# zc402/video-classification

Hardware: AMD Instinct MI355X
Metric: clips/sec SlowFast-R50 8x8, 32x224^2 bf16 training step (higher is better)
Workload: dtype bf16

## Files before the change

### video-classification_amd/csrc/bn_tail.hip

```cpp
#include "sfk_common.h"

namespace {

template <typename D> __device__ __forceinline__ float wload(const void* w, int64_t i) {
  return (float)static_cast<const D*>(w)[i];
}

constexpr int TF_CO = 8;
constexpr int TF_MAXC = 512;

__global__ __launch_bounds__(256) void bn_tail_fold_g_kernel(const float* __restrict__ parts, int nparts, int c, float* __restrict__ g) {
  const int ci = blockIdx.x * 4 + (threadIdx.x >> 6), lane = threadIdx.x & 63;
  if (ci >= c) return;
  double s = 0.0;
  for (int p = lane; p < nparts; p += 64) s += (double)parts[((int64_t)p * c + ci) * 2];
#pragma unroll
  for (int sft = 1; sft < 64; sft <<= 1) s += __shfl_xor(s, sft);
  if (lane == 0) g[ci] = (float)s;
}

template <typename D>
__global__ __launch_bounds__(256) void bn_tail_fwd_kernel(const float* __restrict__ gram, const float* __restrict__ gvec,
                                                          double n, int c, const void* w,
                                                          int cout, const float* gamma, const float* beta, float eps,
                                                          float momentum, float* running_mean, float* running_var,
                                                          int64_t* nbt, float* mean, float* invstd, float* scale,
                                                          float* shift, float* __restrict__ t, D* __restrict__ wd) {
  __shared__ float wl[TF_CO][TF_MAXC];
  __shared__ double gl[TF_MAXC];
  __shared__ double red[4 * TF_CO][2];
  __shared__ float acoef[TF_CO];
  const int co0 = blockIdx.x * TF_CO, tid = threadIdx.x;
  if (blockIdx.x == 0 && tid == 0 && nbt) nbt[0] += 1;
  const double inv_n = 1.0 / n;
  for (int i = tid; i < TF_CO * c; i += 256) {
    const int o = i / c, j = i % c;
    wl[o][j] = co0 + o < cout ? wload<D>(w, (int64_t)(co0 + o) * c + j) : 0.f;
  }
  for (int j = tid; j < c; j += 256) gl[j] = (double)gvec[j] * inv_n;
  __syncthreads();
  constexpr int NR = TF_MAXC / 256;
  float acc[TF_CO][NR], accc[TF_CO][NR];
  double gbar[NR];
#pragma unroll
  for (int r = 0; r < NR; ++r) {
    const int ci = tid + 256 * r;
    gbar[r] = ci < c ? (double)gvec[ci] * inv_n : 0.0;
  }
#pragma unroll
  for (int o = 0; o < TF_CO; ++o)
#pragma unroll
    for (int r = 0; r < NR; ++r) { acc[o][r] = 0.f; accc[o][r] = 0.f; }
#pragma unroll 8
  for (int j = 0; j < c; ++j) {
    float gj[NR], gc[NR];
    const double mj = gl[j];
#pragma unroll
    for (int r = 0; r < NR; ++r) {
      const int ci = tid + 256 * r;
      gj[r] = ci < c ? gram[(int64_t)j * c + ci] : 0.f;
      gc[r] = (float)((double)gj[r] * inv_n - mj * gbar[r]);
    }
#pragma unroll
    for (int o = 0; o < TF_CO; ++o) {
      const float wv = wl[o][j];
#pragma unroll
      for (int r = 0; r < NR; ++r) {
        acc[o][r] += wv * gj[r];
        accc[o][r] += wv * gc[r];
      }
    }
  }
  double p1[TF_CO], p2[TF_CO];
#pragma unroll
  for (int o = 0; o < TF_CO; ++o) {
    p1[o] = 0.0;
    p2[o] = 0.0;
#pragma unroll
    for (int r = 0; r < NR; ++r) {
      const int ci = tid + 256 * r;
      if (ci < c) {
        if (co0 + o < cout) t[(int64_t)(co0 + o) * c + ci] = acc[o][r];
        p1[o] += (double)wl[o][ci] * (double)gvec[ci];
        p2[o] += (double)accc[o][r] * (double)wl[o][ci];
      }
    }
#pragma unroll
    for (int sft = 1; sft < 64; sft <<= 1) {
      p1[o] += __shfl_xor(p1[o], sft);
      p2[o] += __shfl_xor(p2[o], sft);
    }
  }
  if ((tid & 63) == 0) {
#pragma unroll
    for (int o = 0; o < TF_CO; ++o) {
      red[(tid >> 6) * TF_CO + o][0] = p1[o];
      red[(tid >> 6) * TF_CO + o][1] = p2[o];
    }
  }
  __syncthreads();
  if (tid < TF_CO && co0 + tid < cout) {
    const int ch = co0 + tid;
    const double s1 = red[tid][0] + red[TF_CO + tid][0] + red[2 * TF_CO + tid][0] + red[3 * TF_CO + tid][0];
    const double s2 = red[tid][1] + red[TF_CO + tid][1] + red[2 * TF_CO + tid][1] + red[3 * TF_CO + tid][1];
    const double mu = s1 / n;
    double var = s2;
    if (var < 0.0) var = 0.0;
    const float is = (float)(1.0 / sqrt(var + (double)eps));
    const float sc = gamma[ch] * is;
    mean[ch] = (float)mu;
    invstd[ch] = is;
    scale[ch] = sc;
    shift[ch] = beta[ch] - (float)mu * sc;
    acoef[tid] = sc;
    if (running_mean) {
      const double unb = n > 1.0 ? var * n / (n - 1.0) : var;
      running_mean[ch] = (1.f - momentum) * running_mean[ch] + momentum * (float)mu;
      running_var[ch] = (1.f - momentum) * running_var[ch] + momentum * (float)unb;
    }
  }
  if (!wd) return;
  __syncthreads();
  for (int ci = tid; ci < c; ci += 256)
#pragma unroll
    for (int o = 0; o < TF_CO; ++o)
      if (co0 + o < cout) wd[(int64_t)ci * cout + co0 + o] = (D)(acoef[o] * wl[o][ci]);
}

template <typename D>
__global__ __launch_bounds__(256) void bn_tail_coef_kernel(const float* __restrict__ rx, const float* __restrict__ parts,
                                                           int nparts, double n, int c,
                                                           const void* w, int cout, const float* gamma,
                                                           const float* mean, const float* invstd, float* dgamma,
                                                           float* dbeta, float* coef) {
  const int co = blockIdx.x * 4 + (threadIdx.x >> 6), lane = threadIdx.x & 63;
  if (co >= cout) return;
  double sdy = 0.0;
#pragma unroll 4
  for (int ci = lane; ci < c; ci += 64) sdy += (double)wload<D>(w, (int64_t)co * c + ci) * (double)rx[(int64_t)co * c + ci];
  double s = 0.0;
#pragma unroll 8
  for (int p = lane; p < nparts; p += 64) s += (double)parts[((int64_t)p * cout + co) * 2];
#pragma unroll
  for (int sft = 1; sft < 64; sft <<= 1) {
    sdy += __shfl_xor(sdy, sft);
    s += __shfl_xor(s, sft);
  }
  if (lane != 0) return;
  const double is = (double)invstd[co], mu = (double)mean[co];
  const double sxh = is * (sdy - mu * s);
  dgamma[co] += (float)sxh;
  dbeta[co] += (float)s;
  const double A = (double)gamma[co] * is, c1 = s / n, c2 = sxh / n;
  coef[co * 4 + 0] = (float)A;
  coef[co * 4 + 1] = (float)(-A * c2 * is);
  coef[co * 4 + 2] = (float)(A * (c2 * is * mu - c1));
  coef[co * 4 + 3] = 0.f;
}

template <typename D>
__device__ __forceinline__ void bn_tail_apply_part(int bx, int by, const float* __restrict__ rx, const float* __restrict__ gvec,
                                                   const float* __restrict__ t, int c, int cout,
                                                   const float* __restrict__ coef, float* dw) {
  const int co0 = by * 32, ci0 = bx * 32;
  const int tx = threadIdx.x & 31, ty = threadIdx.x >> 5;
#pragma unroll
  for (int i = 0; i < 4; ++i) {
    const int co = co0 + ty + 8 * i, ci = ci0 + tx;
    if (co < cout && ci < c) {
      const float A = coef[co * 4], B = coef[co * 4 + 1], Cc = coef[co * 4 + 2];
      const int64_t idx = (int64_t)co * c + ci;
      dw[idx] += A * rx[idx] + B * t[idx] + Cc * gvec[ci];
    }
  }
}

template <typename D>
__device__ __forceinline__ void bn_tail_m_part(int bx, int by, const void* w, int c, int cout, const float* __restrict__ coef, D* m) {
  __shared__ float wi[16][17], wj[16][17], bco[16];
  const int tx = threadIdx.x & 15, ty = threadIdx.x >> 4;
  const int i = by * 16 + ty, j = bx * 16 + tx;
  float acc = 0.f;
  for (int co0 = 0; co0 < cout; co0 += 16) {
    const int co = co0 + ty;
    const int ci = by * 16 + tx, cj = bx * 16 + tx;
    wi[ty][tx] = (co < cout && ci < c) ? wload<D>(w, (int64_t)co * c + ci) : 0.f;
    wj[ty][tx] = (co < cout && cj < c) ? wload<D>(w, (int64_t)co * c + cj) : 0.f;
    if (threadIdx.x < 16) bco[threadIdx.x] = co0 + threadIdx.x < cout ? coef[(co0 + threadIdx.x) * 4 + 1] : 0.f;
    __syncthreads();
#pragma unroll
    for (int q = 0; q < 16; ++q) acc += bco[q] * wi[q][ty] * wj[q][tx];
    __syncthreads();
  }
  if (i < c && j < c) m[(int64_t)i * c + j] = (D)acc;
}

template <typename D>
__device__ __forceinline__ void bn_tail_bias_part(int bx, const void* w, int c, int cout, const float* __restrict__ coef,
                                                  float* bias) {
  __shared__ double red[16][17];
  const int col = threadIdx.x & 15, part = threadIdx.x >> 4;
  const int ci = bx * 16 + col;
  double s = 0.0;
  if (ci < c) {
#pragma unroll 4
    for (int co = part; co < cout; co += 16) s += (double)coef[co * 4 + 2] * (double)wload<D>(w, (int64_t)co * c + ci);
  }
  red[part][col] = s;
  __syncthreads();
  if (part == 0 && ci < c) {
    double a = 0.0;
#pragma unroll
    for (int p = 0; p < 16; ++p) a += red[p][col];
    bias[ci] = (float)a;
  }
}

template <typename D>
__global__ __launch_bounds__(256) void bn_tail_post_kernel(const float* rx, const float* gvec, const float* t, int c,
                                                           const void* w, int cout, const float* coef, float* dw, D* m,
                                                           float* bias, int ax, int nap, int mx, int nm) {
  int b = blockIdx.x;
  if (b < nap) { bn_tail_apply_part<D>(b % ax, b / ax, rx, gvec, t, c, cout, coef, dw); return; }
  b -= nap;
  if (b < nm) { bn_tail_m_part<D>(b % mx, b / mx, w, c, cout, coef, m); return; }
  bn_tail_bias_part<D>(b - nm, w, c, cout, coef, bias);
}

inline bool tail_args_ok(int c, int cout, int dtype) {
  return c > 0 && cout > 0 && (dtype == SFK_F32 || dtype == SFK_BF16);
}

}

extern "C" int sfk_bn_tail_fwd(const float* gram, const float* a_sums, int32_t a_nparts, int64_t count, float* g, int32_t c,
                               const void* w, int32_t w_dtype, int32_t cout,
                               const float* gamma, const float* beta, float eps, float momentum, float* running_mean,
                               float* running_var, int64_t* nbt, float* mean, float* invstd, float* scale, float* shift,
                               float* t, void* wd, sfk_stream_t stream) {
  if (!gram || !a_sums || a_nparts <= 0 || count <= 0 || !g || !w || !gamma || !beta || !mean || !invstd || !scale || !shift || !t)
    return SFK_ERR_INVALID;
  if (!tail_args_ok(c, cout, w_dtype) || (!running_mean) != (!running_var)) return SFK_ERR_INVALID;
  if (c > TF_MAXC) return SFK_ERR_UNSUPPORTED;
  hipStream_t s = static_cast<hipStream_t>(stream);
  hipLaunchKernelGGL(bn_tail_fold_g_kernel, dim3((c + 3) / 4), dim3(256), 0, s, a_sums, a_nparts, c, g);
  const dim3 grid((cout + TF_CO - 1) / TF_CO), blk(256);
  if (w_dtype == SFK_BF16)
    hipLaunchKernelGGL(bn_tail_fwd_kernel<bf16_t>, grid, blk, 0, s, gram, g, (double)count, c, w, cout, gamma, beta, eps, momentum,
                       running_mean, running_var, nbt, mean, invstd, scale, shift, t, static_cast<bf16_t*>(wd));
  else
    hipLaunchKernelGGL(bn_tail_fwd_kernel<float>, grid, blk, 0, s, gram, g, (double)count, c, w, cout, gamma, beta, eps, momentum,
                       running_mean, running_var, nbt, mean, invstd, scale, shift, t, static_cast<float*>(wd));
  SFK_CHECK_LAUNCH();
  return SFK_OK;
}

template <typename D>
static int tail_bwd_launch(const float* rx, const float* parts, int nparts, const float* g, int64_t count, const float* t, int c, const void* w, int cout,
                           const float* gamma, const float* mean, const float* invstd, float* dgamma, float* dbeta,
                           float* dw, void* m, float* bias, float* coef, hipStream_t s) {
  hipLaunchKernelGGL(bn_tail_coef_kernel<D>, dim3((cout + 3) / 4), dim3(256), 0, s, rx, parts, nparts, (double)count, c, w, cout, gamma, mean,
                     invstd, dgamma, dbeta, coef);
  const int ax = (c + 31) / 32, ay = (cout + 31) / 32, mx = (c + 15) / 16, nb = (c + 15) / 16;
  hipLaunchKernelGGL(bn_tail_post_kernel<D>, dim3(ax * ay + mx * mx + nb), dim3(256), 0, s, rx, g, t, c, w, cout, coef, dw,
                     static_cast<D*>(m), bias, ax, ax * ay, mx, mx * mx);
  SFK_CHECK_LAUNCH();
  return SFK_OK;
}

extern "C" int sfk_bn_tail_bwd(const float* rx, const float* parts, int32_t nparts, const float* g, int64_t count, const float* t,
                               int32_t c, const void* w, int32_t w_dtype, int32_t cout, const float* gamma, const float* mean, const float* invstd,
                               float* dgamma, float* dbeta, float* dw, void* m, float* bias, float* coef,
                               sfk_stream_t stream) {
  if (!rx || !parts || nparts <= 0 || !g || count <= 0 || !t || !w || !gamma || !mean || !invstd || !dgamma || !dbeta || !dw || !m || !bias || !coef)
    return SFK_ERR_INVALID;
  if (!tail_args_ok(c, cout, w_dtype)) return SFK_ERR_INVALID;
  hipStream_t s = static_cast<hipStream_t>(stream);
  return w_dtype == SFK_BF16
             ? tail_bwd_launch<bf16_t>(rx, parts, nparts, g, count, t, c, w, cout, gamma, mean, invstd, dgamma, dbeta, dw, m, bias, coef, s)
             : tail_bwd_launch<float>(rx, parts, nparts, g, count, t, c, w, cout, gamma, mean, invstd, dgamma, dbeta, dw, m, bias, coef, s);
}
```

Before: 1173.

## Fuse partial-sum fold into BN tail forward kernel and stage gram slabs in LDS

The forward tail kernel now folds the per-part channel sums itself when the part count is small, which removes a separate kernel launch. It stages the gram matrix through LDS in slabs with register prefetch, and uses dynamic shared memory with templated column groupings so smaller channel counts keep more threads busy. The backward coef kernel uses a shared fold routine, and the M-part kernel processes 64 output channels per tile instead of 16. Explicit fma and unfused operations pin down rounding, and the code grows more complex with more template variants.

New measurement: 1177, median of 6. About the same (+0.3%).

```diff
diff --git a/video-classification_amd/csrc/bn_tail.hip b/video-classification_amd/csrc/bn_tail.hip
--- a/video-classification_amd/csrc/bn_tail.hip
+++ b/video-classification_amd/csrc/bn_tail.hip
@@ -6,8 +6,59 @@
   return (float)static_cast<const D*>(w)[i];
 }
 
+__device__ __forceinline__ float unfused_mul_add(float a, float b, float c) {
+#pragma clang fp contract(off)
+  const float p = a * b;
+  return c + p;
+}
+__device__ __forceinline__ float unfused_add(float a, float b) {
+#pragma clang fp contract(off)
+  return a + b;
+}
+
 constexpr int TF_CO = 8;
 constexpr int TF_MAXC = 512;
+constexpr int TF_SLAB = 2048;
+constexpr int TF_FOLD_CW = 64;
+
+template <int CW>
+__device__ __forceinline__ void fold_rows(const float* __restrict__ parts, int nparts, int ld, int col0, int ncols, double* red) {
+  static_assert(CW >= 4 && CW <= TF_FOLD_CW && (CW & (CW - 1)) == 0, "column chunk");
+  constexpr int NG = 256 / CW, L = 64 / NG, UNR = 16 / L;
+  const int tid = threadIdx.x, tx = tid % CW, lg = tid / CW;
+  double a[L];
+#pragma unroll
+  for (int i = 0; i < L; ++i) a[i] = 0.0;
+  if (tx < ncols) {
+    const float* base = parts + (int64_t)(col0 + tx) * 2;
+    for (int p0 = lg * L; p0 < nparts; p0 += 64 * UNR) {
+      float v[UNR][L];
+#pragma unroll
+      for (int u = 0; u < UNR; ++u)
+#pragma unroll
+        for (int i = 0; i < L; ++i) {
+          const int p = p0 + 64 * u + i;
+          const float x = base[(int64_t)(p < nparts ? p : nparts - 1) * ld * 2];
+          v[u][i] = p < nparts ? x : 0.f;
+        }
+#pragma unroll
+      for (int u = 0; u < UNR; ++u)
+#pragma unroll
+        for (int i = 0; i < L; ++i) a[i] += (double)v[u][i];
+    }
+  }
+#pragma unroll
+  for (int st = 1; st < L; st <<= 1)
+#pragma unroll
+    for (int i = 0; i < L; i += 2 * st) a[i] += a[i + st];
+  red[tid] = a[0];
+  __syncthreads();
+#pragma unroll
+  for (int st = 1; st < NG; st <<= 1) {
+    if ((lg & (2 * st - 1)) == 0) red[tid] += red[tid + st * CW];
+    __syncthreads();
+  }
+}
 
 __global__ __launch_bounds__(256) void bn_tail_fold_g_kernel(const float* __restrict__ parts, int nparts, int c, float* __restrict__ g) {
   const int ci = blockIdx.x * 4 + (threadIdx.x >> 6), lane = threadIdx.x & 63;
@@ -18,105 +69,162 @@
   for (int sft = 1; sft < 64; sft <<= 1) s += __shfl_xor(s, sft);
   if (lane == 0) g[ci] = (float)s;
 }
-
-template <typename D>
-__global__ __launch_bounds__(256) void bn_tail_fwd_kernel(const float* __restrict__ gram, const float* __restrict__ gvec,
-                                                          double n, int c, const void* w,
+inline bool tail_fold_inside(int c, int nparts) { return (int64_t)c * nparts <= 32 * 256; }
+
+template <typename D, int NO, int NR, int FCW>
+__global__ __launch_bounds__(256) void bn_tail_fwd_kernel(const float* __restrict__ gram, const float* __restrict__ parts,
+                                                          int nparts, float* gout, double n, int c, const void* w,
                                                           int cout, const float* gamma, const float* beta, float eps,
                                                           float momentum, float* running_mean, float* running_var,
                                                           int64_t* nbt, float* mean, float* invstd, float* scale,
                                                           float* shift, float* __restrict__ t, D* __restrict__ wd) {
-  __shared__ float wl[TF_CO][TF_MAXC];
-  __shared__ double gl[TF_MAXC];
-  __shared__ double red[4 * TF_CO][2];
-  __shared__ float acoef[TF_CO];
+  constexpr int CW = 32 * NO;
+  static_assert(NR == 1 || NO == TF_CO, "two register columns only with one group");
+  extern __shared__ double lds[];
+  const int ldw = c + 1;
+  const int rows = c < TF_SLAB / c ? c : TF_SLAB / c;
+  double* gl = lds;
+  double* fred = gl + c;
+  double (*red)[4][2] = reinterpret_cast<double (*)[4][2]>(fred + 256);
+  float* wl_ = reinterpret_cast<float*>(fred + 256 + TF_CO * 4 * 2);
+  float* gs = wl_ + TF_CO * ldw;
+  float* sg = gs + c;
+  float* sc = sg + rows * c;
+  float* acoef = sc + rows * c;
+  auto wl = [&](int o, int j) -> float& { return wl_[o * ldw + j]; };
   const int co0 = blockIdx.x * TF_CO, tid = threadIdx.x;
+  const int tx = tid % CW, grp = tid / CW;
   if (blockIdx.x == 0 && tid == 0 && nbt) nbt[0] += 1;
   const double inv_n = 1.0 / n;
+  float pre[TF_SLAB / 256];
+  auto fetch = [&](int j0) {
+    const int nelem = (c - j0 < rows ? c - j0 : rows) * c;
+    const float* src = gram + (int64_t)j0 * c;
+#pragma unroll
+    for (int u = 0; u < TF_SLAB / 256; ++u) {
+      const int e = tid + 256 * u;
+      pre[u] = src[e < nelem ? e : 0];
+    }
+  };
+  fetch(0);
   for (int i = tid; i < TF_CO * c; i += 256) {
     const int o = i / c, j = i % c;
-    wl[o][j] = co0 + o < cout ? wload<D>(w, (int64_t)(co0 + o) * c + j) : 0.f;
-  }
-  for (int j = tid; j < c; j += 256) gl[j] = (double)gvec[j] * inv_n;
-  __syncthreads();
-  constexpr int NR = TF_MAXC / 256;
-  float acc[TF_CO][NR], accc[TF_CO][NR];
-  double gbar[NR];
-#pragma unroll
-  for (int r = 0; r < NR; ++r) {
-    const int ci = tid + 256 * r;
-    gbar[r] = ci < c ? (double)gvec[ci] * inv_n : 0.0;
-  }
-#pragma unroll
-  for (int o = 0; o < TF_CO; ++o)
-#pragma unroll
-    for (int r = 0; r < NR; ++r) { acc[o][r] = 0.f; accc[o][r] = 0.f; }
-#pragma unroll 8
-  for (int j = 0; j < c; ++j) {
-    float gj[NR], gc[NR];
-    const double mj = gl[j];
+    const float wv = wload<D>(w, (int64_t)(co0 + o < cout ? co0 + o : cout - 1) * c + j);
+    wl(o, j) = co0 + o < cout ? wv : 0.f;
+  }
+  if (tid < TF_CO * 4 * 2) fred[256 + tid] = 0.0;
+  if (parts) {
+    for (int c0 = 0; c0 < c; c0 += FCW) {
+      const int nc = c - c0 < FCW ? c - c0 : FCW;
+      fold_rows<FCW>(parts, nparts, c, c0, nc, fred);
+      if (tid < nc) {
+        const float gv = (float)fred[tid];
+        gs[c0 + tid] = gv;
+        gl[c0 + tid] = (double)gv * inv_n;
+        if (blockIdx.x == 0) gout[c0 + tid] = gv;
+      }
+      __syncthreads();
+    }
+  } else {
+    for (int j = tid; j < c; j += 256) {
+      const float gv = gout[j];
+      gs[j] = gv;
+      gl[j] = (double)gv * inv_n;
+    }
+    __syncthreads();
+  }
+  float acc[NO][NR], accc[NO][NR];
+#pragma unroll
+  for (int k = 0; k < NO; ++k)
+#pragma unroll
+    for (int r = 0; r < NR; ++r) { acc[k][r] = 0.f; accc[k][r] = 0.f; }
+  const int sq = 256 / c, sr = 256 % c;
+  int col[NR];
+#pragma unroll
+  for (int r = 0; r < NR; ++r) col[r] = tx + 256 * r < c ? tx + 256 * r : 0;
+  for (int j0 = 0; j0 < c;) {
+    const int nrow = c - j0 < rows ? c - j0 : rows, nelem = nrow * c;
+    int jj = tid / c, ci = tid - jj * c;
+#pragma unroll
+    for (int u = 0; u < TF_SLAB / 256; ++u) {
+      const int e = tid + 256 * u;
+      if (e < nelem) {
+        sg[e] = pre[u];
+        sc[e] = (float)__builtin_fma((double)pre[u], inv_n, -(gl[j0 + jj] * gl[ci]));
+      }
+      jj += sq;
+      ci += sr;
+      if (ci >= c) { ci -= c; ++jj; }
+    }
+    __syncthreads();
+    const int jn = j0 + nrow;
+    if (jn < c) fetch(jn);
+#pragma unroll 4
+    for (int jj = 0; jj < nrow; ++jj) {
+      float gj[NR], gc[NR];
+#pragma unroll
+      for (int r = 0; r < NR; ++r) {
+        gj[r] = sg[jj * c + col[r]];
+        gc[r] = sc[jj * c + col[r]];
+      }
+#pragma unroll
+      for (int k = 0; k < NO; ++k) {
+        const float wv = wl(grp * NO + k, j0 + jj);
+#pragma unroll
+        for (int r = 0; r < NR; ++r) {
+          acc[k][r] = __builtin_fmaf(wv, gj[r], acc[k][r]);
+          accc[k][r] = __builtin_fmaf(wv, gc[r], accc[k][r]);
+        }
+      }
+    }
+    __syncthreads();
+    j0 = jn;
+  }
+#pragma unroll
+  for (int k = 0; k < NO; ++k) {
+    const int o = grp * NO + k;
+    double p1 = 0.0, p2 = 0.0;
 #pragma unroll
     for (int r = 0; r < NR; ++r) {
-      const int ci = tid + 256 * r;
-      gj[r] = ci < c ? gram[(int64_t)j * c + ci] : 0.f;
-      gc[r] = (float)((double)gj[r] * inv_n - mj * gbar[r]);
-    }
-#pragma unroll
-    for (int o = 0; o < TF_CO; ++o) {
-      const float wv = wl[o][j];
-#pragma unroll
-      for (int r = 0; r < NR; ++r) {
-        acc[o][r] += wv * gj[r];
-        accc[o][r] += wv * gc[r];
-      }
-    }
-  }
-  double p1[TF_CO], p2[TF_CO];
-#pragma unroll
-  for (int o = 0; o < TF_CO; ++o) {
-    p1[o] = 0.0;
-    p2[o] = 0.0;
-#pragma unroll
-    for (int r = 0; r < NR; ++r) {
-      const int ci = tid + 256 * r;
+      const int ci = tx + 256 * r;
       if (ci < c) {
-        if (co0 + o < cout) t[(int64_t)(co0 + o) * c + ci] = acc[o][r];
-        p1[o] += (double)wl[o][ci] * (double)gvec[ci];
-        p2[o] += (double)accc[o][r] * (double)wl[o][ci];
-      }
-    }
-#pragma unroll
-    for (int sft = 1; sft < 64; sft <<= 1) {
-      p1[o] += __shfl_xor(p1[o], sft);
-      p2[o] += __shfl_xor(p2[o], sft);
-    }
-  }
-  if ((tid & 63) == 0) {
-#pragma unroll
-    for (int o = 0; o < TF_CO; ++o) {
-      red[(tid >> 6) * TF_CO + o][0] = p1[o];
-      red[(tid >> 6) * TF_CO + o][1] = p2[o];
+        if (co0 + o < cout) t[(int64_t)(co0 + o) * c + ci] = acc[k][r];
+        p1 += (double)wl(o, ci) * (double)gs[ci];
+        p2 += (double)accc[k][r] * (double)wl(o, ci);
+      }
+    }
+#pragma unroll
+    for (int sft = 1; sft < 32; sft <<= 1) {
+      p1 += __shfl_xor(p1, sft);
+      p2 += __shfl_xor(p2, sft);
+    }
+    const double u1 = __shfl_xor(p1, 32), u2 = __shfl_xor(p2, 32);
+    p1 += CW >= 64 ? u1 : 0.0;
+    p2 += CW >= 64 ? u2 : 0.0;
+    if ((tx & 63) == 0) {
+      red[o][tx >> 6][0] = p1;
+      red[o][tx >> 6][1] = p2;
     }
   }
   __syncthreads();
   if (tid < TF_CO && co0 + tid < cout) {
     const int ch = co0 + tid;
-    const double s1 = red[tid][0] + red[TF_CO + tid][0] + red[2 * TF_CO + tid][0] + red[3 * TF_CO + tid][0];
-    const double s2 = red[tid][1] + red[TF_CO + tid][1] + red[2 * TF_CO + tid][1] + red[3 * TF_CO + tid][1];
+    const double s1 = red[tid][0][0] + red[tid][1][0] + red[tid][2][0] + red[tid][3][0];
+    const double s2 = red[tid][0][1] + red[tid][1][1] + red[tid][2][1] + red[tid][3][1];
     const double mu = s1 / n;
     double var = s2;
     if (var < 0.0) var = 0.0;
     const float is = (float)(1.0 / sqrt(var + (double)eps));
-    const float sc = gamma[ch] * is;
+    const float sc_ = gamma[ch] * is;
     mean[ch] = (float)mu;
     invstd[ch] = is;
-    scale[ch] = sc;
-    shift[ch] = beta[ch] - (float)mu * sc;
-    acoef[tid] = sc;
+    scale[ch] = sc_;
+    shift[ch] = __builtin_fmaf(-sc_, (float)mu, beta[ch]);
+    acoef[tid] = sc_;
     if (running_mean) {
       const double unb = n > 1.0 ? var * n / (n - 1.0) : var;
-      running_mean[ch] = (1.f - momentum) * running_mean[ch] + momentum * (float)mu;
-      running_var[ch] = (1.f - momentum) * running_var[ch] + momentum * (float)unb;
+      running_mean[ch] = unfused_add((1.f - momentum) * running_mean[ch], momentum * (float)mu);
+      running_var[ch] = __builtin_fmaf(momentum, (float)unb, (1.f - momentum) * running_var[ch]);
     }
   }
   if (!wd) return;
@@ -124,8 +232,10 @@
   for (int ci = tid; ci < c; ci += 256)
 #pragma unroll
     for (int o = 0; o < TF_CO; ++o)
-      if (co0 + o < cout) wd[(int64_t)ci * cout + co0 + o] = (D)(acoef[o] * wl[o][ci]);
-}
+      if (co0 + o < cout) wd[(int64_t)ci * cout + co0 + o] = (D)(acoef[o] * wl(o, ci));
+}
+
+constexpr int TC_CO = 4;
 
 template <typename D>
 __global__ __launch_bounds__(256) void bn_tail_coef_kernel(const float* __restrict__ rx, const float* __restrict__ parts,
@@ -133,29 +243,36 @@
                                                            const void* w, int cout, const float* gamma,
                                                            const float* mean, const float* invstd, float* dgamma,
                                                            float* dbeta, float* coef) {
-  const int co = blockIdx.x * 4 + (threadIdx.x >> 6), lane = threadIdx.x & 63;
-  if (co >= cout) return;
-  double sdy = 0.0;
+  __shared__ double fred[256];
+  const int co0 = blockIdx.x * TC_CO, lane = threadIdx.x & 63, wave = threadIdx.x >> 6;
+  double sdy[TC_CO / 4];
+#pragma unroll
+  for (int k = 0; k < TC_CO / 4; ++k) {
+    const int co = co0 + wave + 4 * k;
+    sdy[k] = 0.0;
+    if (co < cout) {
 #pragma unroll 4
-  for (int ci = lane; ci < c; ci += 64) sdy += (double)wload<D>(w, (int64_t)co * c + ci) * (double)rx[(int64_t)co * c + ci];
-  double s = 0.0;
-#pragma unroll 8
-  for (int p = lane; p < nparts; p += 64) s += (double)parts[((int64_t)p * cout + co) * 2];
-#pragma unroll
-  for (int sft = 1; sft < 64; sft <<= 1) {
-    sdy += __shfl_xor(sdy, sft);
-    s += __shfl_xor(s, sft);
-  }
-  if (lane != 0) return;
-  const double is = (double)invstd[co], mu = (double)mean[co];
-  const double sxh = is * (sdy - mu * s);
-  dgamma[co] += (float)sxh;
-  dbeta[co] += (float)s;
-  const double A = (double)gamma[co] * is, c1 = s / n, c2 = sxh / n;
-  coef[co * 4 + 0] = (float)A;
-  coef[co * 4 + 1] = (float)(-A * c2 * is);
-  coef[co * 4 + 2] = (float)(A * (c2 * is * mu - c1));
-  coef[co * 4 + 3] = 0.f;
+      for (int ci = lane; ci < c; ci += 64) sdy[k] += (double)wload<D>(w, (int64_t)co * c + ci) * (double)rx[(int64_t)co * c + ci];
+    }
+  }
+  fold_rows<TC_CO>(parts, nparts, cout, co0, cout - co0 < TC_CO ? cout - co0 : TC_CO, fred);
+#pragma unroll
+  for (int k = 0; k < TC_CO / 4; ++k) {
+    const int co = co0 + wave + 4 * k;
+#pragma unroll
+    for (int sft = 1; sft < 64; sft <<= 1) sdy[k] += __shfl_xor(sdy[k], sft);
+    if (lane != 0 || co >= cout) continue;
+    const double s = fred[wave + 4 * k];
+    const double is = (double)invstd[co], mu = (double)mean[co];
+    const double sxh = is * __builtin_fma(-mu, s, sdy[k]);
+    dgamma[co] += (float)sxh;
+    dbeta[co] += (float)s;
+    const double A = (double)gamma[co] * is, c1 = s / n, c2 = sxh / n;
+    coef[co * 4 + 0] = (float)A;
+    coef[co * 4 + 1] = (float)(-A * c2 * is);
+    coef[co * 4 + 2] = (float)(A * __builtin_fma(c2 * is, mu, -c1));
+    coef[co * 4 + 3] = 0.f;
+  }
 }
 
 template <typename D>
@@ -170,26 +287,38 @@
     if (co < cout && ci < c) {
       const float A = coef[co * 4], B = coef[co * 4 + 1], Cc = coef[co * 4 + 2];
       const int64_t idx = (int64_t)co * c + ci;
-      dw[idx] += A * rx[idx] + B * t[idx] + Cc * gvec[ci];
-    }
-  }
-}
-
+      dw[idx] = unfused_add(dw[idx], unfused_add(__builtin_fmaf(A, rx[idx], B * t[idx]), Cc * gvec[ci]));
+    }
+  }
+}
+
+constexpr int TM_CO = 64;
 template <typename D>
 __device__ __forceinline__ void bn_tail_m_part(int bx, int by, const void* w, int c, int cout, const float* __restrict__ coef, D* m) {
-  __shared__ float wi[16][17], wj[16][17], bco[16];
+  __shared__ float wi[TM_CO][17], wj[TM_CO][17], bco[TM_CO];
   const int tx = threadIdx.x & 15, ty = threadIdx.x >> 4;
   const int i = by * 16 + ty, j = bx * 16 + tx;
+  const int ci = by * 16 + tx, cj = bx * 16 + tx;
   float acc = 0.f;
-  for (int co0 = 0; co0 < cout; co0 += 16) {
-    const int co = co0 + ty;
-    const int ci = by * 16 + tx, cj = bx * 16 + tx;
-    wi[ty][tx] = (co < cout && ci < c) ? wload<D>(w, (int64_t)co * c + ci) : 0.f;
-    wj[ty][tx] = (co < cout && cj < c) ? wload<D>(w, (int64_t)co * c + cj) : 0.f;
-    if (threadIdx.x < 16) bco[threadIdx.x] = co0 + threadIdx.x < cout ? coef[(co0 + threadIdx.x) * 4 + 1] : 0.f;
-    __syncthreads();
-#pragma unroll
-    for (int q = 0; q < 16; ++q) acc += bco[q] * wi[q][ty] * wj[q][tx];
+  for (int co0 = 0; co0 < cout; co0 += TM_CO) {
+#pragma unroll
+    for (int u = 0; u < TM_CO / 16; ++u) {
+      const int co = co0 + ty + 16 * u;
+      const int64_t row = (int64_t)(co < cout ? co : cout - 1) * c;
+      const float vi = wload<D>(w, row + (ci < c ? ci : c - 1)), vj = wload<D>(w, row + (cj < c ? cj : c - 1));
+      wi[ty + 16 * u][tx] = (co < cout && ci < c) ? vi : 0.f;
+      wj[ty + 16 * u][tx] = (co < cout && cj < c) ? vj : 0.f;
+    }
+    if (threadIdx.x < TM_CO) bco[threadIdx.x] = co0 + threadIdx.x < cout ? coef[(co0 + threadIdx.x) * 4 + 1] : 0.f;
+    __syncthreads();
+    const int nq = cout - co0 < TM_CO ? (cout - co0 + 15) & ~15 : TM_CO;
+    for (int q0 = 0; q0 < nq; q0 += 16) {
+#pragma unroll
+      for (int q = 0; q < 16; ++q) {
+        const float bw = bco[q0 + q] * wi[q0 + q][ty];
+        acc = q < 4 ? __builtin_fmaf(bw, wj[q0 + q][tx], acc) : unfused_mul_add(bw, wj[q0 + q][tx], acc);
+      }
+    }
     __syncthreads();
   }
   if (i < c && j < c) m[(int64_t)i * c + j] = (D)acc;
@@ -229,6 +358,25 @@
 
 inline bool tail_args_ok(int c, int cout, int dtype) {
   return c > 0 && cout > 0 && (dtype == SFK_F32 || dtype == SFK_BF16);
+}
+
+inline size_t tail_fwd_lds(int c) {
+  const int rows = c < TF_SLAB / c ? c : TF_SLAB / c;
+  return sizeof(double) * (c + 256 + TF_CO * 4 * 2) + sizeof(float) * (TF_CO * (c + 1) + c + 2 * rows * c + TF_CO);
+}
+template <typename D, int NO, int NR, int FCW, typename... A>
+void tail_fwd_launch1(int c, dim3 grid, hipStream_t s, A... a) {
+  hipLaunchKernelGGL((bn_tail_fwd_kernel<D, NO, NR, FCW>), grid, dim3(256), tail_fwd_lds(c), s, a...);
+}
+template <typename D, typename... A>
+void tail_fwd_launch(int c, dim3 grid, hipStream_t s, A... a) {
+  if (c > 256) tail_fwd_launch1<D, 8, 2, 64>(c, grid, s, a...);
+  else if (c > 128) tail_fwd_launch1<D, 8, 1, 64>(c, grid, s, a...);
+  else if (c > 64) tail_fwd_launch1<D, 4, 1, 64>(c, grid, s, a...);
+  else if (c > 32) tail_fwd_launch1<D, 2, 1, 64>(c, grid, s, a...);
+  else if (c > 16) tail_fwd_launch1<D, 1, 1, 32>(c, grid, s, a...);
+  else if (c > 8) tail_fwd_launch1<D, 1, 1, 16>(c, grid, s, a...);
+  else tail_fwd_launch1<D, 1, 1, 8>(c, grid, s, a...);
 }
 
 }
@@ -243,14 +391,17 @@
   if (!tail_args_ok(c, cout, w_dtype) || (!running_mean) != (!running_var)) return SFK_ERR_INVALID;
   if (c > TF_MAXC) return SFK_ERR_UNSUPPORTED;
   hipStream_t s = static_cast<hipStream_t>(stream);
-  hipLaunchKernelGGL(bn_tail_fold_g_kernel, dim3((c + 3) / 4), dim3(256), 0, s, a_sums, a_nparts, c, g);
-  const dim3 grid((cout + TF_CO - 1) / TF_CO), blk(256);
+  const dim3 grid((cout + TF_CO - 1) / TF_CO);
+  if (!tail_fold_inside(c, a_nparts)) {
+    hipLaunchKernelGGL(bn_tail_fold_g_kernel, dim3((c + 3) / 4), dim3(256), 0, s, a_sums, a_nparts, c, g);
+    a_sums = nullptr;
+  }
   if (w_dtype == SFK_BF16)
-    hipLaunchKernelGGL(bn_tail_fwd_kernel<bf16_t>, grid, blk, 0, s, gram, g, (double)count, c, w, cout, gamma, beta, eps, momentum,
-                       running_mean, running_var, nbt, mean, invstd, scale, shift, t, static_cast<bf16_t*>(wd));
+    tail_fwd_launch<bf16_t>(c, grid, s, gram, a_sums, (int)a_nparts, g, (double)count, (int)c, w, (int)cout, gamma, beta, eps, momentum,
+                            running_mean, running_var, nbt, mean, invstd, scale, shift, t, static_cast<bf16_t*>(wd));
   else
-    hipLaunchKernelGGL(bn_tail_fwd_kernel<float>, grid, blk, 0, s, gram, g, (double)count, c, w, cout, gamma, beta, eps, momentum,
-                       running_mean, running_var, nbt, mean, invstd, scale, shift, t, static_cast<float*>(wd));
+    tail_fwd_launch<float>(c, grid, s, gram, a_sums, (int)a_nparts, g, (double)count, (int)c, w, (int)cout, gamma, beta, eps, momentum,
+                           running_mean, running_var, nbt, mean, invstd, scale, shift, t, static_cast<float*>(wd));
   SFK_CHECK_LAUNCH();
   return SFK_OK;
 }
@@ -259,8 +410,8 @@
 static int tail_bwd_launch(const float* rx, const float* parts, int nparts, const float* g, int64_t count, const float* t, int c, const void* w, int cout,
                            const float* gamma, const float* mean, const float* invstd, float* dgamma, float* dbeta,
                            float* dw, void* m, float* bias, float* coef, hipStream_t s) {
-  hipLaunchKernelGGL(bn_tail_coef_kernel<D>, dim3((cout + 3) / 4), dim3(256), 0, s, rx, parts, nparts, (double)count, c, w, cout, gamma, mean,
-                     invstd, dgamma, dbeta, coef);
+  hipLaunchKernelGGL(bn_tail_coef_kernel<D>, dim3((cout + TC_CO - 1) / TC_CO), dim3(256), 0, s, rx, parts, nparts, (double)count, c, w, cout,
+                     gamma, mean, invstd, dgamma, dbeta, coef);
   const int ax = (c + 31) / 32, ay = (cout + 31) / 32, mx = (c + 15) / 16, nb = (c + 15) / 16;
   hipLaunchKernelGGL(bn_tail_post_kernel<D>, dim3(ax * ay + mx * mx + nb), dim3(256), 0, s, rx, g, t, c, w, cout, coef, dw,
                      static_cast<D*>(m), bias, ax, ax * ay, mx, mx * mx);
```
